# vghuy17ck1/svt-av1-psyex

Hardware: AMD Instinct MI355X
Metric: ME+RD-cost Mpixels/s (2160p10 preset-6) (higher is better)
Workload: dtype u8 SAD / i32 transforms; 1 GPU; 3840x2160 10-bit synthetic pan sequence, preset 6 (M6) search controls at qp 35; step = 16 pictures (4 current pictures x ref distance 1,2,4,8; R=2): open-loop ME of all 2040 b64 + full-pel pred + RD chain (64x64,32x32,16x16 DCT_DCT, 10-bit, b quantizer; qcoeff + recon + scalars written); 3 picture sets alternate from step to step

## Files before the change

svt-av1-psyex_amd/csrc/me_kernel.hip:

```cpp
#include <hip/hip_runtime.h>
#include <stdint.h>
#include <string.h>
#include "me_kernel.h"
#include "wave_ops.h"
#include "lds_dma.h"

#ifdef SVT_HIP_ME_PROFILE
struct Prof { uint32_t *acc; unsigned long long last; int step; };
#define SVT_HIP_ME_PROFILE_LDS (48 * 4)
#define PROF_DECL Prof prof_; prof_.acc = reinterpret_cast<uint32_t *>(g_lds + lay.total); if (threadIdx.x < 48) prof_.acc[threadIdx.x] = 0; prof_.last = __builtin_readcyclecounter(); prof_.step = 0; Prof *prof = &prof_
#define PROF_STEP(s) (prof->step = (s))
#define PROFS(i) PROF((i) + prof->step)
#define PROF(i) do { const unsigned long long t_ = __builtin_readcyclecounter(); if (threadIdx.x == 0) atomicAdd(&prof->acc[i], (uint32_t)(t_ - prof->last)); prof->last = t_; } while (0)
#define PROF_FLUSH(ptr) do { __builtin_amdgcn_fence(__ATOMIC_RELEASE, "wavefront"); if (threadIdx.x < 48) atomicAdd((unsigned long long *)(ptr) + threadIdx.x, (unsigned long long)prof->acc[threadIdx.x]); } while (0)
#define PROF_PARAM , Prof *prof
#define PROF_ARG , prof
#else
#define PROF_DECL do { } while (0)
#define PROF(i) do { } while (0)
#define PROFS(i) do { } while (0)
#define PROF_STEP(s) do { } while (0)
#define PROF_FLUSH(ptr) do { } while (0)
#define SVT_HIP_ME_PROFILE_LDS 0
#define PROF_PARAM
// ... 506 lines not shown
    constexpr int kArenaVec = kWinBytes / 16;
    int nt = 1;
    if (n1 <= kSmallVec && n0 + n1 <= kArenaVec) {
        nt = 2;
        if (n2 <= kSmallVec && n0 + n1 + n2 <= kArenaVec) {
            nt = 3;
            if (n3 <= kSmallVec && n0 + n1 + n2 + n3 <= kArenaVec) nt = 4;
        }
    }
    tile_load<0, 2>(read_tile(st, i), v);
    if (nt > 1) tile_load<2, 2>(read_tile(st, i + 1), v);
    if (nt > 2) tile_load<4, 2>(read_tile(st, i + 2), v);
    if (nt > 3) tile_load<6, 2>(read_tile(st, i + 3), v);
    return nt;
}
static_assert(kVecPerLane >= 8, "four small tiles of two slots each");

__device__ __forceinline__ void run_searches(Shared &sh PROF_PARAM) {
    St        &st   = sh.st;
    const int  nreq = (int)uni((uint32_t)st.nreq);
    V4         v[kVecPerLane];
    u64        key = (0xffffffull << 32) | 0xffffffffull;
    for (int t0 = 0;; t0 += kMaxTiles) {
        const int total = plan_tiles(st, nreq, t0), n = imin(total - t0, kMaxTiles);
        wave_sync();
        int nv[4] = {0, 0, 0, 0}, nvn[4] = {0, 0, 0, 0};
        int i = 0, nt = load_round(st, 0, n, v, nv);
        PROFS(24);
        while (nt) {
            {
                if (nv[0] > kSmallVec) tile_store<0, kVecPerLane>(sh, nv[0], 0, v);
                else {
                    tile_store<0, 2>(sh, nv[0], 0, v);
                    if (nt > 1) tile_store<2, 2>(sh, nv[1], nv[0], v);
                    if (nt > 2) tile_store<4, 2>(sh, nv[2], nv[0] + nv[1], v);
                    if (nt > 3) tile_store<6, 2>(sh, nv[3], nv[0] + nv[1] + nv[2], v);
                }
            }
            wave_sync();
            PROFS(32);
            const int nn = load_round(st, i + nt, n, v, nvn);
            PROF(22);
            int lds_vec = 0;
            for (int j = 0; j < nt; j++) {
                const TileGeo t = read_tile(st, i + j);
                const u64 k = tile_eval(sh, t, lds_vec * 16 PROF_ARG);
                key = k < key ? k : key;
                lds_vec += t.nvec;
                if (t.last) {
                    if (threadIdx.x == 0) st.req_key[t.req] = key;
                    key = (0xffffffull << 32) | 0xffffffffull;
                }
            }
            wave_sync();
            PROFS(40);
            i += nt;
            nt = nn;
#pragma unroll
            for (int j = 0; j < 4; j++) nv[j] = nvn[j];
        }
        if (t0 + kMaxTiles >= total) break;
        wave_sync();
    }
}

template <int NDW, int DEPTH>
__device__ __forceinline__ void direct_rows(uint8_t *arena, const uint8_t *src, int sp, int srs, const uint8_t *wp, long long wstep, int e0, int rows, int rows_max, uint32_t out[8]) {
    constexpr int NV = (NDW + 2 + 3) / 4, kRowsPerFlush = 64 / NDW;
    static_assert(NV & 1, "owners read their pieces back without bank conflicts");
    static_assert(DEPTH >= 1 && DEPTH <= 3, "steps in flight");
    const int lane = threadIdx.x;
    const uint8_t *pp[NV];
    int            pn[NV];
#pragma unroll
    for (int k = 0; k < NV; k++) {
        const int n = lane + 64 * k, owner = n / NV, part = n - owner * NV;
        const u64 base = ((u64)(uint32_t)__shfl((int)(uint32_t)((uintptr_t)wp >> 32), owner, 64) << 32) | (uint32_t)__shfl((int)(uint32_t)(uintptr_t)wp, owner, 64);
        pp[k] = reinterpret_cast<const uint8_t *>((uintptr_t)base) + 16 * part;
        pn[k] = __shfl(rows, owner, 64);
    }
    uint32_t a[8] = {0, 0, 0, 0, 0, 0, 0, 0};
    V4U v[DEPTH][NV];
    auto request = [&](V4U (&r)[NV], int step) {
#pragma unroll
        for (int k = 0; k < NV; k++) {
            if (step < pn[k]) r[k] = *reinterpret_cast<GV4U *>(reinterpret_cast<uintptr_t>(pp[k]));
            pp[k] += wstep;
        }
    };
#pragma unroll
    for (int dpt = 0; dpt < DEPTH; dpt++) {
#pragma unroll
        for (int k = 0; k < NV; k++) v[dpt][k] = V4U{0, 0, 0, 0};
        request(v[dpt], dpt);
    }
    u64 acc0 = 0, acc1 = 0;
    auto step = [&](V4U (&r)[NV], int t) {
#pragma unroll
        for (int k = 0; k < NV; k++) *reinterpret_cast<V4U *>(arena + 16 * (lane + 64 * k)) = r[k];
        wave_sync();
        request(r, t + DEPTH);
        if (t < rows) {
            const uint32_t *s = reinterpret_cast<const uint32_t *>(src + (e0 + t) * srs * sp);
            uint32_t sv[NDW], wv[4 * NV];
#pragma unroll
            for (int j = 0; j < NDW; j += 4) {
                const uint4 q = *reinterpret_cast<const uint4 *>(s + j);
                sv[j] = q.x; sv[j + 1] = q.y; sv[j + 2] = q.z; sv[j + 3] = q.w;
            }
#pragma unroll
            for (int k = 0; k < NV; k++) {
                const uint4 q = *reinterpret_cast<const uint4 *>(arena + 16 * (lane * NV + k));
                wv[4 * k] = q.x; wv[4 * k + 1] = q.y; wv[4 * k + 2] = q.z; wv[4 * k + 3] = q.w;
            }
#pragma unroll
            for (int j = 0; j < NDW; j++) {
                acc0 = __builtin_amdgcn_qsad_pk_u16_u8(((u64)wv[j + 1] << 32) | wv[j], sv[j], acc0);
                acc1 = __builtin_amdgcn_qsad_pk_u16_u8(((u64)wv[j + 2] << 32) | wv[j + 1], sv[j], acc1);
            }
        }
        if ((t + 1) % kRowsPerFlush == 0 || t + 1 == rows_max) {
#pragma unroll
            for (int i = 0; i < 4; i++) { a[i] += (uint32_t)((acc0 >> (16 * i)) & 0xFFFF); a[4 + i] += (uint32_t)((acc1 >> (16 * i)) & 0xFFFF); }
            acc0 = acc1 = 0;
        }
        wave_sync();
    };
    for (int t = 0; t < rows_max; t += DEPTH) {
        step(v[0], t);
        if (DEPTH >= 2 && t + 1 < rows_max) step(v[DEPTH >= 2 ? 1 : 0], t + 1);
        if (DEPTH >= 3 && t + 2 < rows_max) step(v[DEPTH >= 3 ? 2 : 0], t + 2);
    }
#pragma unroll
    for (int i = 0; i < 8; i++) out[i] = a[i];
}

__device__ __forceinline__ bool small_direct_ok(const St &st, int *q_total = nullptr) {
    const int lane = threadIdx.x, nreq = (int)uni((uint32_t)st.nreq);
    const Req &r0 = st.req[0];
    const int  bw = (int)uni(r0.bw), bh = (int)uni(r0.bh), rs = (int)uni(r0.rs), level = (int)uni(r0.level), stride = (int)uni((uint32_t)r0.stride);
    bool ok = true;
    int  per = 0;
    if (lane < nreq) {
        const Req &r = st.req[lane];
        const int  w = r.sa_w, h = r.sa_h;
        ok  = w > 0 && h > 0 && w * h <= kNarrowMaxPos && r.bw == bw && r.bh == bh && r.rs == rs && r.level == level && (int)r.stride == stride && !r.skip_even && !r.done;
        per = ((w + 7) >> 3) * h;
    }
    if (!__all(ok) || (bw != 32 && bw != 64) || nreq > kMaxReq || nreq <= 0) return false;
    const int q = (int)wave_sum_dpp((uint32_t)per);
    if (q_total) *q_total = q;
    return q <= kThreads;
}
template <int DEPTH = 1> __device__ __forceinline__ bool run_small_searches_direct(Shared &sh PROF_PARAM) {
    St       &st   = sh.st;
    const int lane = threadIdx.x, nreq = (int)uni((uint32_t)st.nreq);
    int Q = 0;
    if (!small_direct_ok(st, &Q)) return false;
    Q = (int)uni((uint32_t)Q);
    const Req &r0 = st.req[0];
    const int  bw = (int)uni(r0.bw), bh = (int)uni(r0.bh), rs = (int)uni(r0.rs), level = (int)uni(r0.level);
    {
        int per = 0;
        if (lane < nreq) per = ((st.req[lane].sa_w + 7) >> 3) * st.req[lane].sa_h;
        int incl = per;
#pragma unroll
        for (int o = 1; o < 32; o <<= 1) { const int t = __shfl_up(incl, o, 64); if ((lane & 31) >= o) incl += t; }
        if (lane < nreq) st.req_key[lane] = (u64)(uint32_t)(incl - per);
    }
    wave_sync();
    int       S        = imin(bh, (int)uni(div_by_rcp((uint32_t)kThreads, rcp_of((uint32_t)Q))));
    const int rows_per = (int)uni(div_by_rcp((uint32_t)(bh + S - 1), rcp_of((uint32_t)S)));
    S                  = (int)uni(div_by_rcp((uint32_t)(bh + rows_per - 1), rcp_of((uint32_t)rows_per)));
    uint32_t *sad = reinterpret_cast<uint32_t *>(LDS(sh.win));
    const uint8_t *src = src_view(sh, level);
    const int      sp  = (level == 2) ? kSrc64Pitch : (level == 1 ? kSrc32Pitch : kSrc16Pitch), srs = rs >> sh.cshift;
    const long long wstep = (long long)rs * (long long)(int)uni((uint32_t)r0.stride);
    const bool mine = lane < Q * S;
    int req = 0, y = 0, g = 0, e0 = 0, rows = 0, w = 1;
    const uint8_t *wp = nullptr;
    if (mine) {
        const int slice = (int)div_by_rcp((uint32_t)lane, rcp_of((uint32_t)Q)), q = lane - slice * Q;
        for (int r = 1; r < nreq; r++) req += q >= (int)(uint32_t)st.req_key[r] ? 1 : 0;
        const Req &r = st.req[req];
        w = r.sa_w;
        const int ng = (w + 7) >> 3, ql = q - (int)(uint32_t)st.req_key[req];
        y = (int)div_by_rcp((uint32_t)ql, rcp_of((uint32_t)ng)); g = ql - y * ng;
        e0   = slice * rows_per;
        rows = imin(e0 + rows_per, bh) - e0;
        wp   = r.win + (long long)y * r.stride + (long long)e0 * wstep + 8 * g;
    }
    uint32_t s8[8];
    PROF(26);
    if (bw == 64) direct_rows<16, DEPTH>(LDS(sh.win), src, sp, srs, wp, wstep, e0, rows, rows_per, s8);
    else direct_rows<8, DEPTH>(LDS(sh.win), src, sp, srs, wp, wstep, e0, rows, rows_per, s8);
    PROF(27);
    for (int p = lane; p < nreq * kNarrowMaxPos; p += kThreads) sad[p] = 0;
    wave_sync();
    if (mine) {
#pragma unroll
        for (int i = 0; i < 8; i++)
            if (8 * g + i < w) atomicAdd(&sad[req * kNarrowMaxPos + y * w + 8 * g + i], s8[i]);
    }
    wave_sync();
    PROF(23);
    for (int rq = 0; rq < nreq; rq++) {
        const int      wr = (int16_t)uni((uint32_t)st.req[rq].sa_w), hr = (int16_t)uni((uint32_t)st.req[rq].sa_h);
        const uint32_t k32 = wave_min_dpp(lane < wr * hr ? (sad[rq * kNarrowMaxPos + lane] << 6) | (uint32_t)lane : 0xFFFFFFFFu);
        const int      wl = (int)(k32 & 63u), wy = (int)uni(div_by_rcp((uint32_t)wl, rcp_of((uint32_t)wr))), wx = wl - wy * wr;
        if (lane == 0) st.req_key[rq] = ((u64)(k32 >> 6) << 32) | ((uint32_t)wy << 16) | (uint32_t)wx;
    }
    wave_sync();
    return true;
}

constexpr int kDenseKinds = SVT_HIP_ME_DENSE_KINDS;
__device__ __forceinline__ uint32_t dense_pack(int a, int b) { return (uint32_t)(uint16_t)a | ((uint32_t)(uint16_t)b << 16); }
__device__ __forceinline__ void dense_take(St &st, const MeDenseSlot *dl, int idx, int req, const SearchGeo &g, uint32_t &n_hit, uint32_t &n_miss) {
    if (!dl) return;
    const MeDenseSlot s = dl[idx];
    if (s.org == dense_pack(g.ox, g.oy) && s.size == dense_pack(g.sa_w, g.sa_h)) {
        st.req[req].done = 1;
        st.req_key[req]  = s.key == ~0ull ? ((0xffffffull << 32) | 0xffffffffull) : s.key;
        n_hit++;
    } else
        n_miss++;
}

__device__ __forceinline__ void push_req(St &st, const uint8_t *win, uint32_t stride, int sa_w, int sa_h, int bw, int bh, int rs,
                                         int level, int skip, int slot = -1) {
    Req &r      = st.req[slot >= 0 ? slot : st.nreq++];
    r.win       = win;
    r.stride    = stride;
    r.sa_w      = (int16_t)sa_w;
    r.sa_h      = (int16_t)sa_h;
    r.bw        = (uint8_t)bw;
    r.bh        = (uint8_t)bh;
    r.rs        = (uint8_t)rs;
    r.level     = (uint8_t)level;
    r.skip_even = (uint8_t)(skip && bw == 16 && bh <= 16);
    r.done      = 0;
}

__device__ __forceinline__ void push_hme_req(St &st, CParams &p, int level, CPlane &rp, int org_x, int org_y,
                                             int bw, int bh, int ox, int oy, int sa_w, int sa_h, int skip, int slot = -1) {
    const int full = (p.cfg.hme_search_method == 1);
    push_req(st, plane_at(rp, org_x + ox, org_y + oy), rp.stride, sa_w, sa_h, bw, full ? bh : (bh >> 1), full ? 1 : 2, level, skip, slot);
}


__device__ __forceinline__ void upd(u64 &best, uint32_t sad, uint32_t ord) {
    const u64 k = ((u64)sad << 32) | ord;
    best        = k < best ? k : best;
}

__device__ __attribute__((noinline)) void stage_clamped(uint8_t *win, const uint8_t *pix0, uint32_t stride, int min_x, int max_x, int min_y, int max_y, int wx0, int wy0,
                                                        int pitch, int rows) {
    for (int i = threadIdx.x; i < pitch * rows; i += kThreads) {
        const int row = i / pitch, cb = i - row * pitch;
        const int x = imin(imax(wx0 + cb, min_x), max_x), y = imin(imax(wy0 + row, min_y), max_y);
        win[row * pitch + cb] = pix0[x + (long long)y * stride];
    }
}

constexpr int kMeOrdBits = 12;
__device__ __forceinline__ void run_me_searches(Shared &sh, CParams &p, const MeReq *list, int count, uint32_t *bsad, uint32_t *bmv, int r0n PROF_PARAM) {
    const int lane = threadIdx.x;
    const int sub  = (p.cfg.me_search_method == 0);
    const int nrow = sub ? 4 : 8, rstep = sub ? 2 : 1;
    const int g = lane >> 4, pu = lane & 15;
    const int bx = (pu & 1) | ((pu >> 1) & 2), by = ((pu >> 1) & 1) | ((pu >> 2) & 2);
    const uint8_t *srow = &LDS(sh.src64)[bx * 16];
    for (int mi = 0; mi < count; mi++) {
        MeReq m;
        {
            const MeReq &mm = list[mi];
            m.pix0 = uni_ptr(mm.pix0); m.stride = uni(mm.stride);
            m.ox = (int16_t)uni((uint32_t)mm.ox); m.oy = (int16_t)uni((uint32_t)mm.oy); m.sa_w = (int16_t)uni((uint32_t)mm.sa_w); m.sa_h = (int16_t)uni((uint32_t)mm.sa_h);
            m.li = (uint8_t)uni(mm.li); m.ri = (uint8_t)uni(mm.ri); m.probe = 0; m.pad = 0;
            m.min_x = (int16_t)uni((uint32_t)mm.min_x); m.max_x = (int16_t)uni((uint32_t)mm.max_x); m.min_y = (int16_t)uni((uint32_t)mm.min_y); m.max_y = (int16_t)uni((uint32_t)mm.max_y);
        }
        u64 b8[4] = {~0ull, ~0ull, ~0ull, ~0ull}, b16 = ~0ull, b32 = ~0ull, b64 = ~0ull;
        const int W = m.sa_w, H = m.sa_h;
        int       tw = W, th = H;
        auto me_pitch = [](int shift, int ww) { return ((shift + ww - 1 + 64 + 15) & ~15) + 16; };
        auto wbytes = [&](int ww, int hh) { return (uint32_t)me_pitch(0, ww) * (uint32_t)(hh - 1 + 64); };
        while (th > 1 && (wbytes(tw, th) > (uint32_t)kWinBytes || tw * th > (1 << kMeOrdBits))) th = (th + 1) >> 1;
        while (tw > 8 && (wbytes(tw, th) > (uint32_t)kWinBytes || tw * th > (1 << kMeOrdBits))) tw = ((tw >> 1) + 7) & ~7;
        for (int y0 = 0; y0 < H; y0 += th)
            for (int x0 = 0; x0 < W; x0 += tw) {
                const int w = imin(tw, W - x0), h = imin(th, H - y0);
                const uint8_t *gwin  = m.pix0 + (m.ox + x0) + (long long)(m.oy + y0) * m.stride;
                const int pitch = me_pitch(0, w);
                const int rows        = h - 1 + 64;
                const int vec_per_row = pitch >> 4;
                lds_dma_after_stores();
                const int wx0 = m.ox + x0, wy0 = m.oy + y0;
                if (m.ox + x0 >= m.min_x && m.ox + x0 + w - 1 + 63 <= m.max_x && wy0 >= m.min_y && wy0 + rows - 1 <= m.max_y) {
                    lds_dma_window(gwin, m.stride, vec_per_row, rows, g_lds, sh.win);
                    lds_dma_wait();
                } else {
                    stage_clamped(LDS(sh.win), m.pix0, m.stride, m.min_x, m.max_x, m.min_y, m.max_y, wx0, wy0, pitch, rows);
                }
                wave_sync();
                PROF(46);
                const int ng = (w + 3) >> 2;
                uint32_t k8[4] = {~0u, ~0u, ~0u, ~0u}, k16 = ~0u, k32 = ~0u, k64 = ~0u;
                const int kshift = kMeOrdBits + sub;
                for (int y = 0; y < h; y += 4) {
                    const bool live = y + g < h;
                    const int  yy   = live ? y + g : h - 1;
                    const uint8_t *wrow = &LDS(sh.win)[(yy + by * 16) * pitch + bx * 16];
                    const uint32_t ord0 = (uint32_t)(yy * w);
                    for (int gq = 0; gq < ng; gq++) {
                        const uint8_t *wp = wrow + 4 * gq;
                        u64 acc[4] = {0, 0, 0, 0};
#pragma unroll
// ... 275 lines not shown
    else { y = (int)((key >> 16) & 0xFFFF); x = (int)(key & 0xFFFF); }
    if (!full) sad *= 2;
}

__device__ __forceinline__ void push_zz_req(St &st, CPlane &rp, int dx, int dy, int slot = -1) {
    push_req(st, plane_at(rp, (int)st.org_x + dx, (int)st.org_y + dy), rp.stride, 1, 1, (int)st.b64_w, (int)st.b64_h >> 1, 2, 2, 0, slot);
}

}


#ifndef SVT_ME_CTRL_PRIO
#define SVT_ME_CTRL_PRIO 2
#endif
#define CTRL_PRIO(x) __builtin_amdgcn_s_setprio(x)

constexpr size_t kPersistBytes = (offsetof(St, req) + 15) & ~(size_t)15;
template <int MODE>
__device__ __forceinline__ void me_b64_body(const MeBatchHeader *__restrict__ ghdr, const MeKernelParams *__restrict__ gparams, const uint32_t launch_flags) {
    St     &st = *reinterpret_cast<St *>(g_lds);
    constexpr bool kImports = MODE == kMeMid2 || MODE == kMeTail;
    typedef const SVT_CONST_AS MeBatchHeader CHeader;
    CHeader  &hdr = *(CHeader *)ghdr;
    const int tid = threadIdx.x;
    const int       cshift = (int)hdr.cshift;
    const bool      has_dense = hdr.dense != nullptr;
    const LdsLayout lay    = lds_layout((int)hdr.n_slot, cshift, has_dense ? 1 : 0, MODE);
    uint32_t *const bsad = reinterpret_cast<uint32_t *>(g_lds + lay.bsad);
    uint32_t *const bmv  = reinterpret_cast<uint32_t *>(g_lds + lay.bmv);
    const MeDenseSlot *const dense_lds = has_dense ? reinterpret_cast<const MeDenseSlot *>(g_lds + lay.dense) : nullptr;
    uint32_t n_hit = 0, n_miss = 0;
    Shared sh = {st, lay.src64, lay.src32, lay.src16, lay.win, cshift};

    uint32_t xcc = 0;
    asm volatile("s_getreg_b32 %0, hwreg(HW_REG_XCC_ID)" : "=s"(xcc));
    xcc &= 7;
    int queue_probe = 0;
    constexpr int kList = 0;
    const bool list_mode = (launch_flags & 1u) != 0;
    const uint32_t n_total = hdr.job_base[hdr.n_pictures];
    uint32_t share_next = 0, share_end = 0, share_step = 1;
    if (MODE != kMeFull && !list_mode) {
        if (gridDim.x >= SVT_HIP_ME_QUEUES) {
            const uint32_t q = blockIdx.x % SVT_HIP_ME_QUEUES;
            share_step = (gridDim.x - q + SVT_HIP_ME_QUEUES - 1) / SVT_HIP_ME_QUEUES;
            share_next = hdr.queue_begin[q] + blockIdx.x / SVT_HIP_ME_QUEUES;
            share_end  = hdr.queue_begin[q + 1];
        } else {
            share_step = gridDim.x; share_next = blockIdx.x; share_end = n_total;
        }
    }
    auto fetch_job = [&]() {
        int job = -1;
        if (list_mode) {
            const uint32_t n = __hip_atomic_load(&hdr.queue_head[SVT_HIP_ME_LIST_COUNT(kList)], __ATOMIC_RELAXED, __HIP_MEMORY_SCOPE_AGENT);
            if (__hip_atomic_load(&hdr.queue_head[SVT_HIP_ME_LIST_CURSOR(kList)], __ATOMIC_RELAXED, __HIP_MEMORY_SCOPE_AGENT) >= n) return job;
            const uint32_t k = atomicAdd(&hdr.queue_head[SVT_HIP_ME_LIST_CURSOR(kList)], 1u);
            if (k < n) job = (int)hdr.lists[kList][k];
            return job;
        }
        if (MODE != kMeFull) {
            if (share_next < share_end) { job = (int)share_next; share_next += share_step; }
            return job;
        }
        while (queue_probe < SVT_HIP_ME_QUEUES) {
            const int      q  = (int)((xcc + queue_probe) & 7);
            const uint32_t lo = hdr.queue_begin[q], hi = hdr.queue_begin[q + 1];
            if (lo < hi) {
                const uint32_t k = atomicAdd(&hdr.queue_head[q], 1u);
                if (lo + k < hi) { job = (int)(lo + k); break; }
            }
            queue_probe++;
        }
        return job;
    };
    auto stage_base = [&](int gjob) { return hdr.stage + (size_t)gjob * SVT_HIP_ME_STAGE_BYTES; };
    auto export_state = [&](int gjob) {
        uint4 *dst = reinterpret_cast<uint4 *>(stage_base(gjob));
        const uint4 *src = reinterpret_cast<const uint4 *>(g_lds);
        for (int i = tid; i < (int)(kPersistBytes / 16); i += kThreads) dst[i] = src[i];
    };
    static_assert(kPersistBytes + kMaxReq * (sizeof(Req) + sizeof(u64)) <= SVT_HIP_ME_STAGE_BYTES, "a block's record holds its state, its requests and their results");
    auto export_reqs = [&](int gjob) {
        uint4 *dst = reinterpret_cast<uint4 *>(stage_base(gjob) + kPersistBytes);
        const uint4 *src = reinterpret_cast<const uint4 *>(st.req);
        static_assert(sizeof(Req) == 24 && (kMaxReq * sizeof(Req)) % 16 == 0, "requests are copied as 16-byte words");
        for (int i = tid; i < (int)(kMaxReq * sizeof(Req) / 16); i += kThreads) dst[i] = src[i];
    };
    auto keys_of = [&](int gjob) { return reinterpret_cast<u64 *>(stage_base(gjob) + kPersistBytes + kMaxReq * sizeof(Req)); };
    PROF_DECL;

    for (;;) {
        int gjob = 0;
        if (tid == 0) gjob = fetch_job();
        gjob = __builtin_amdgcn_readfirstlane(gjob);
        if (gjob < 0) break;
        PROF(0);
        int pic = 0;
        while (pic + 1 < (int)hdr.n_pictures && (uint32_t)gjob >= hdr.job_base[pic + 1]) pic++;
        pic = __builtin_amdgcn_readfirstlane(pic);
        CParams &p = ((CParams *)gparams)[pic];
        auto &c = p.cfg;
        auto &d = p.desc;
        const int full_hme = (c.hme_search_method == 1);
        const int nl       = d.num_of_list_to_search;
        const bool mctf    = c.me_type == 1;
        const int job      = gjob - (int)hdr.job_base[pic];
        const uint32_t bxi = (uint32_t)job % p.w64, byi = p.row0 + (uint32_t)job / p.w64;
        const uint32_t b   = bxi + byi * p.w64;
        const int r0n      = d.num_of_ref_pic_to_search[0];
#define BEST_SAD(li, ri) (bsad + (((li) ? r0n : 0) + (ri)) * 85)
#define BEST_MV(li, ri) (bmv + (((li) ? r0n : 0) + (ri)) * 85)
        const int n_rows   = r0n + (nl > 1 ? d.num_of_ref_pic_to_search[1] : 0);
        uint32_t *const jflag = hdr.job_flags ? hdr.job_flags + gjob : nullptr;
        if constexpr (me_is_search(MODE)) {
            constexpr int lvl = MODE == kMeS1 ? 1 : 2, parts = lvl == 1 ? 3 : 5;
            static_assert(offsetof(St, req) == kPersistBytes && offsetof(St, nreq) >= kPersistBytes - 16, "nreq sits in the last 16-byte word of the record's head, the requests behind it");
            static_assert(kSrc32Pitch == 3 * 16 && kSrc64Pitch == 5 * 16, "a view row is its pieces and one piece of padding");
            lds_dma_after_stores();
            lds_dma_copy(stage_base(gjob) + kPersistBytes - 16, g_lds, (uint32_t)(kPersistBytes - 16), 1 + (int)(kMaxReq * sizeof(Req) / 16));
            const int ox = (int)(bxi * 64) >> (2 - lvl), oy = (int)(byi * 64) >> (2 - lvl), rstep = 1 << cshift, npiece = ((lvl == 1 ? 32 : 64) >> cshift) * parts;
            for (int b0 = 0; b0 < npiece; b0 += kThreads) {
                const int n = b0 + tid, row = n / parts, cc = n - row * parts;
                if (n < npiece && cc < parts - 1) lds_dma_load16(plane_at(p.cur.lvl[lvl], ox + cc * 16, oy + row * rstep), g_lds, (lvl == 1 ? lay.src32 : lay.src64) + (uint32_t)b0 * 16);
            }
            const uint32_t f = __hip_atomic_load(jflag, __ATOMIC_RELAXED, __HIP_MEMORY_SCOPE_AGENT);
            lds_dma_wait();
            if (f & SVT_HIP_ME_JOB_DEFERRED) continue;
        } else if constexpr (kImports) {
            static_assert(offsetof(St, req_key) % 16 == 0 && kPersistBytes <= offsetof(St, req) + 8 && offsetof(St, req) + 8 <= offsetof(St, req_key), "the record's parts land on 16-byte words of their own");
            static_assert(kSrc64Pitch == 5 * 16, "a view row is four pieces and one piece of padding");
            lds_dma_after_stores();
            lds_dma_copy(stage_base(gjob), g_lds, 0, (int)(kPersistBytes / 16));
            lds_dma_copy(reinterpret_cast<const uint8_t *>(keys_of(gjob)), g_lds, (uint32_t)offsetof(St, req_key), (int)(kMaxReq * sizeof(u64) / 16));
            if constexpr (MODE == kMeTail) {
                const int ox = (int)(bxi * 64), oy = (int)(byi * 64), rstep = 1 << cshift, npiece = (64 >> cshift) * 5;
                for (int b0 = 0; b0 < npiece; b0 += kThreads) {
                    const int n = b0 + tid, row = n / 5, cc = n - row * 5;
                    if (n < npiece && cc < 4) lds_dma_load16(plane_at(p.cur.lvl[2], ox + cc * 16, oy + row * rstep), g_lds, lay.src64 + (uint32_t)b0 * 16);
                }
            }
            const uint32_t f = __hip_atomic_load(jflag, __ATOMIC_RELAXED, __HIP_MEMORY_SCOPE_AGENT);
            if constexpr (MODE == kMeTail)
                for (int i = tid; i < n_rows * 85; i += kThreads) { bmv[i] = 0; bsad[i] = SVT_HIP_MAX_SAD_VALUE; }
            if (tid == 0) { st.nme = 0; st.nprobe = 0; }
            lds_dma_wait();
            if (f & SVT_HIP_ME_JOB_DEFERRED) continue;
        }
        if constexpr (me_is_search(MODE)) {
            PROF(24);
            wave_sync();
            PROF(25);
            if (st.nreq) {
                (void)run_small_searches_direct<SVT_HIP_ME_SEARCH_DEPTH>(sh PROF_ARG);
            }
            wave_sync();
            u64 *keys = keys_of(gjob);
            if (tid < kMaxReq) keys[tid] = st.req_key[tid];
            wave_sync();
            continue;
        }

        if constexpr (!kImports) {
        if (tid == 0) {
            st.b64_index = b;
            st.org_x = bxi * 64; st.org_y = byi * 64;
            st.b64_w = (uint32_t)(d.aligned_width - st.org_x) < 64 ? d.aligned_width - st.org_x : 64;
            st.b64_h = (uint32_t)(d.aligned_height - st.org_y) < 64 ? d.aligned_height - st.org_y : 64;
            st.hme_l0_sa.sa_min.width = (uint16_t)c.hme_l0_sa.sa_min.width; st.hme_l0_sa.sa_min.height = (uint16_t)c.hme_l0_sa.sa_min.height;
            st.hme_l0_sa.sa_max.width = (uint16_t)c.hme_l0_sa.sa_max.width; st.hme_l0_sa.sa_max.height = (uint16_t)c.hme_l0_sa.sa_max.height;
            st.nreq = 0; st.nme = 0; st.nprobe = 0;
        }
        for (int i = tid; i < 3 * 2 * 4 * 2 * 2; i += kThreads) { (&st.hx[0][0][0][0][0])[i] = 0; (&st.hy[0][0][0][0][0])[i] = 0; (&st.hs[0][0][0][0][0])[i] = 0; }
        if constexpr (MODE == kMeFull)
            for (int i = tid; i < n_rows * 85; i += kThreads) { bmv[i] = 0; bsad[i] = SVT_HIP_MAX_SAD_VALUE; }
        if (tid < 8) {
            const int li = tid >> 2, ri = tid & 3;
            st.do_ref[li][ri] = 1; st.hme_sad64[li][ri] = 0xFFFFFFFFull; st.sr_divisor[li][ri] = 1; st.zz_sad[li][ri] = ~0u;
            st.hme_sc_x[li][ri] = st.hme_sc_y[li][ri] = 0;
            for (int sri = 0; sri < 2; sri++) {
                PreHme &ph = st.prehme[li][ri][sri];
                ph.valid = 0; ph.col = ph.row = 0; ph.sad = 0; ph.sa_w = ph.sa_h = 0;
                st.performed_phme[li][ri][sri] = 0;
            }
        }
        }
        if ((MODE == kMeFull || MODE == kMeMid1) && has_dense && tid < n_rows * kDenseKinds)
            reinterpret_cast<uint4 *>(g_lds + lay.dense)[tid] = reinterpret_cast<const uint4 *>(hdr.dense)[((size_t)gjob * hdr.n_slot) * kDenseKinds + tid];
        const bool zz_on = (MODE == kMeFull || MODE == kMeMid1) && (c.me_early_exit_th || c.me_safe_limit_zz_th);
        const int  nzz   = zz_on ? r0n + ((nl > 1 && d.temporal_layer_index > 0) ? d.num_of_ref_pic_to_search[1] : 0) : 0;
        uint32_t   zz_sum[8] = {0, 0, 0, 0, 0, 0, 0, 0};
        {
            const int ox = (int)(bxi * 64), oy = (int)(byi * 64), rstep = 1 << cshift;
            const int bw64 = imin(64, (int)d.aligned_width - ox), bh64 = imin(64, (int)d.aligned_height - oy);
            if constexpr (!kImports)
            for (int i = tid; i < (64 >> cshift) * 4; i += kThreads) {
                const int row = i >> 2, cc = i & 3;
                uint4 v; memcpy(&v, plane_at(p.cur.lvl[2], ox + cc * 16, oy + row * rstep), 16);
                if constexpr (MODE != kMeMid1) *reinterpret_cast<uint4 *>(&LDS(sh.src64)[row * kSrc64Pitch + cc * 16]) = v;
                const int y = row * rstep, x = cc * 16;
                if (nzz && !(y & 1) && y < bh64 && x < bw64) {
                    const bool whole = x + 8 < bw64;
#pragma unroll
                    for (int k = 0; k < 8; k++)
                        if (k < nzz) {
                            const int li = k < r0n ? 0 : 1, ri = k < r0n ? k : k - r0n;
                            uint4 w; memcpy(&w, plane_at(p.ref[li][ri].lvl[2], ox + x, oy + y), 16);
                            uint32_t a = __builtin_amdgcn_sad_u8(v.x, w.x, zz_sum[k]);
                            a = __builtin_amdgcn_sad_u8(v.y, w.y, a);
                            if (whole) { a = __builtin_amdgcn_sad_u8(v.z, w.z, a); a = __builtin_amdgcn_sad_u8(v.w, w.w, a); }
                            zz_sum[k] = a;
                        }
                }
            }
            if constexpr (MODE == kMeFull) {
                for (int i = tid; i < (32 >> cshift) * 2; i += kThreads) {
                    const int row = i >> 1, cc = i & 1;
                    uint4 v; memcpy(&v, plane_at(p.cur.lvl[1], (ox >> 1) + cc * 16, (oy >> 1) + row * rstep), 16);
                    *reinterpret_cast<uint4 *>(&LDS(sh.src32)[row * kSrc32Pitch + cc * 16]) = v;
                }
                for (int i = tid; i < (16 >> cshift); i += kThreads) {
                    uint4 v; memcpy(&v, plane_at(p.cur.lvl[0], ox >> 2, (oy >> 2) + i * rstep), 16);
                    *reinterpret_cast<uint4 *>(&LDS(sh.src16)[i * kSrc16Pitch]) = v;
                }
            }
        }
#pragma unroll
        for (int k = 0; k < 8; k++)
            if (k < nzz) {
                const uint32_t t = wave_sum_dpp(zz_sum[k]);
                if (tid == 0) st.req_key[k] = (u64)t << 32;
            }
        wave_sync();

        PROF(1);
        auto zz_pre = [&]() {
            if (tid == 0) st.nreq = 0;
        };
        auto zz_post = [&]() {
            const int  li = (tid >> 2) & 1, ri = tid & 3;
            const bool valid = tid < 8 && li < nl && ri < d.num_of_ref_pic_to_search[li];
            const bool srch  = valid && searched(p, li);
            const u64  smask = __ballot(srch);
            uint32_t   z = 0xFFFFFFFFu;
            if (srch) {
                const int k = __popcll(smask & ((1ull << tid) - 1ull));
                z = (uint32_t)(st.req_key[k] >> 32) << 1;
                z = (z * 64 * 64) / (st.b64_w * st.b64_h);
                st.zz_sad[li][ri] = z;
            }
            const uint32_t best = wave_min_dpp(z);
            if (d.temporal_layer_index > 0 && best < c.zz_sad_th && valid && ri >= 1)
                if ((uint32_t)((z - best) * 100) > (uint32_t)(c.zz_sad_pct * best)) st.do_ref[li][ri] = 0;
            if (c.me_safe_limit_zz_th) {
                wave_sync();
                const bool limit = d.hierarchical_levels > 0 && nl == 2 && d.temporal_layer_index >= d.hierarchical_levels &&
                    d.similar_brightness_refs && st.zz_sad[0][0] < c.me_safe_limit_zz_th && st.zz_sad[1][0] < c.me_safe_limit_zz_th;
                if (limit && valid && ri >= 1) st.do_ref[li][ri] = 0;
            }
        };
        auto prehme_pre = [&](int bi) {
            const int  l_lo = c.prehme_l1_early_exit ? bi : 0, l_hi = c.prehme_l1_early_exit ? bi + 1 : nl;
            const int  li = (tid >> 3) & 1, ri = (tid >> 1) & 3, sri = tid & 1;
            const bool mine = tid < 16 && li >= l_lo && li < l_hi && ri < d.num_of_ref_pic_to_search[li];
            bool       push = false;
            if (mine) {
                st.ph_req[li][ri][sri] = 0;
                if (searched(p, li)) {
                    PreHme &ph = st.prehme[li][ri][sri];
                    bool    handled = false;
                    if (c.me_early_exit_th && st.zz_sad[li][ri] < c.me_early_exit_th) { ph.col = ph.row = 0; ph.sad = 0; ph.valid = 1; handled = true; }
                    if (!handled && c.prehme_l1_early_exit) {
                        const PreHme &q = st.prehme[0][ri][sri];
                        if (li == 1 && q.valid && (q.sad < 32 * 32 || (iabs(q.col) < 16 && iabs(q.row) < 16))) {
                            ph.col = (int16_t)-q.col; ph.row = (int16_t)-q.row; ph.sad = q.sad; ph.valid = 1; handled = true;
                        }
                    }
                    if (!handled && !st.do_ref[li][ri]) { ph.col = ph.row = 0; ph.sad = 0xFFFFFFFFu; handled = true; }
                    push = !handled;
                }
            }
            const u64 mask = __ballot(push);
            const int slot = __popcll(mask & ((1ull << tid) - 1ull));
            if (push) {
                PreHme &ph = st.prehme[li][ri][sri];
                CPlane &rp = p.ref[li][ri].lvl[0];
                const int ox16 = (int16_t)st.org_x >> 2, oy16 = (int16_t)st.org_y >> 2;
                const SearchGeo sg = prehme_geometry(p, li, ri, sri, st.org_x, st.org_y);
                push_hme_req(st, p, 0, rp, ox16, oy16, (int)st.b64_w >> 2, (int)st.b64_h >> 2, sg.ox, sg.oy, sg.sa_w, sg.sa_h, c.prehme_skip_search_line, slot);
                st.ph_req[li][ri][sri] = (uint8_t)(slot + 1);
                dense_take(st, dense_lds, (((li ? r0n : 0) + ri) * kDenseKinds + sri), slot, sg, n_hit, n_miss);
                ph.col = (int16_t)sg.ox; ph.row = (int16_t)sg.oy;
                st.performed_phme[li][ri][sri] = 1;
            }
            if (tid == 0) st.nreq = __popcll(mask);
        };
        auto prehme_post = [&](int bi) {
            const int  l_lo = c.prehme_l1_early_exit ? bi : 0, l_hi = c.prehme_l1_early_exit ? bi + 1 : nl;
            const int  li = (tid >> 3) & 1, ri = (tid >> 1) & 3, sri = tid & 1;
            const bool mine = tid < 16 && li >= l_lo && li < l_hi && ri < d.num_of_ref_pic_to_search[li];
            const int  k = mine ? st.ph_req[li][ri][sri] : 0;
            if (k) {
                PreHme &ph = st.prehme[li][ri][sri];
                uint32_t sad; int x, y;
                key_to_result(st.req_key[k - 1], full_hme, sad, x, y);
                ph.sad = sad;
                ph.col = (int16_t)((int16_t)(x + ph.col) * 4);
// ... 245 lines not shown
                { const uint32_t q = (uint32_t)(int)sa_w / st.sr_divisor[li][ri]; sa_w = (int16_t)(((q > 1u ? q : 1u) + 7) & ~7u); }
                { const uint32_t q = (uint32_t)(int)sa_h / st.sr_divisor[li][ri]; sa_h = (int16_t)(q > 3u ? q : 3u); }
                const int16_t h0 = sa_h, w0 = sa_w;
                u64 best_hme_sad = ~0ull;
                if (c.me_early_exit_th) {
                    if (st.zz_sad[li][ri] < c.me_early_exit_th / 6) sa_w = sa_h = 1;
                } else {
                    int accurate = 1;
                    const int k2 = st.c00_req[li][ri];
                    if (k2) {
                        const uint32_t zero = (uint32_t)(st.req_key[k2 - 2] >> 32) << 1;
                        const uint32_t hme  = (uint32_t)(st.req_key[k2 - 1] >> 32) << 1;
                        if (zero <= hme) cx = cy = 0;
                        best_hme_sad = hme;
                        if (cx == 0 && cy == 0) accurate = 0;
                    }
                    if (c.enable_me_sr_adjustment == 2) {
                        if ((accurate && best_hme_sad < 24 * 24) || (d.is_ref && st.hme_sad64[li][ri] < 24 * 24)) sa_h = (int16_t)(sa_h / 2);
                        if ((li || ri) && BEST_SAD(0, 0)[0] < 5000 && sa_h == h0 && sa_w == w0) { sa_h = (int16_t)(sa_h >> 1); sa_w = (int16_t)(sa_w >> 1); }
                    }
                }
                m.pix0 = plane_at(rp, (int)st.org_x, (int)st.org_y); m.stride = rp.stride;
                m.min_x = (int16_t)(-rp.org_x - (int)st.org_x); m.max_x = (int16_t)(rp.width + rp.org_x - 1 - (int)st.org_x);
                m.min_y = (int16_t)(-rp.org_y - (int)st.org_y); m.max_y = (int16_t)(rp.height + rp.org_y - 1 - (int)st.org_y);
                m.li = (uint8_t)li; m.ri = (uint8_t)ri; m.pad = 0;
                m.sa_w = sa_w; m.sa_h = sa_h;
                m.ox = cx; m.oy = cy;
                m.probe = (c.me_8x8_var_enabled && sa_w * sa_h > 24) ? 1 : 0;
            }
            const bool probe = mine && m.probe;
            const u64  mask = __ballot(mine), pmask = __ballot(probe), below = (1ull << tid) - 1ull;
            if (mine) st.me[__popcll(mask & below)] = m;
            if (probe) { MeReq pr = m; pr.sa_w = pr.sa_h = 1; st.me_probe[__popcll(pmask & below)] = pr; }
            if (tid == 0) { st.nme = __popcll(mask); st.nprobe = __popcll(pmask); }
        };
        auto main_pre = [&]() {
            if (tid < 64) {
                const int pic_w = (int16_t)d.aligned_width, pic_h = (int16_t)d.aligned_height;
                for (int i = 0; i < st.nme; i++) {
                    const MeReq m = st.me[i];
                    int16_t sa_w = m.sa_w, sa_h = m.sa_h;
                    const int cx = m.ox, cy = m.oy;
                    if (m.probe) {
                        const uint32_t mean = BEST_SAD(m.li, m.ri)[0] / 64;
                        const int32_t  dd   = (int32_t)BEST_SAD(m.li, m.ri)[21 + tid] - (int32_t)mean;
                        const uint32_t var  = wave_sum((uint32_t)(dd * dd)) / 64;
                        if (var > c.me_sr_mult2_th) { sa_w = (int16_t)((imax(1, sa_w * 3 / 2) + 7) & ~7); sa_h = (int16_t)imax(1, sa_h * 3 / 2); }
                        if (var < c.me_sr_div4_th) { sa_w = (int16_t)((imax(1, sa_w >> 2) + 7) & ~7); sa_h = (int16_t)imax(3, imax(1, sa_h >> 2)); }
                        else if (var < c.me_sr_div2_th) { sa_w = (int16_t)((imin(sa_w, sa_w >> 1) + 7) & ~7); sa_h = (int16_t)imax(3, imin(sa_h, sa_h >> 1)); }
                    }
                    int ox = (int16_t)(cx - (sa_w >> 1)), oy = (int16_t)(cy - (sa_h >> 1)), w = sa_w, h = sa_h;
                    clip_axis((int16_t)st.org_x, ox, w, 63, pic_w);
                    w = (w < 8) ? w : (w & ~7);
                    clip_axis((int16_t)st.org_y, oy, h, 63, pic_h);
                    if (tid == 0) { MeReq &o = st.me[i]; o.ox = (int16_t)ox; o.oy = (int16_t)oy; o.sa_w = (int16_t)w; o.sa_h = (int16_t)h; }
                }
            }
        };

        enum { kZz, kPrehme, kL0, kL1, kL2, kC00, kProbe, kMain, kEnd };
#ifdef SVT_ME_ABLATE
        if (SVT_ME_ABLATE == 1) continue;
#endif
        const int n_prehme = c.prehme_l1_early_exit ? nl : 1, n_l0 = l0_dep ? 2 : 1, n_group = me_dep ? 2 : 1;
        if constexpr (MODE == kMeMid1 || MODE == kMeMid2) {
            const bool hme_on = c.enable_hme_flag;
            bool defer = false;
            uint32_t flags = 0;
            if constexpr (MODE == kMeMid1) {
                auto pending = [&]() { return __any(tid < st.nreq && !st.req[tid].done); };
                if (c.me_early_exit_th || c.me_safe_limit_zz_th) { zz_pre(); wave_sync(); zz_post(); wave_sync(); }
                if (c.prehme_enable) {
                    for (int b2 = 0; b2 < n_prehme; b2++) {
                        prehme_pre(b2); wave_sync();
                        if (pending()) { defer = true; break; }
                        prehme_post(b2);
                        if (b2 + 1 < n_prehme) wave_sync();
                    }
                    if (!defer) { prehme_final(); wave_sync(); }
                }
                if (!defer && hme_on && c.enable_hme_level0_flag)
                    for (int b2 = 0; b2 < n_l0; b2++) {
                        l0_pre(b2); wave_sync();
                        if (pending()) { defer = true; break; }
                        l0_post(b2); wave_sync();
                    }
                if (!defer) {
                    if (hme_on && c.enable_hme_level1_flag) lvl_pre(1);
                    else if (tid == 0) st.nreq = 0;
                    wave_sync();
                }
            } else {
                flags = __hip_atomic_load(jflag, __ATOMIC_RELAXED, __HIP_MEMORY_SCOPE_AGENT);
                if (hme_on && c.enable_hme_level1_flag) { lvl_post(1); wave_sync(); }
                if (hme_on && c.enable_hme_level2_flag) lvl_pre(2);
                else if (tid == 0) st.nreq = 0;
                wave_sync();
            }
            if (!defer && st.nreq && !small_direct_ok(st)) defer = true;
            if (defer) {
                if (tid == 0) {
                    *jflag = SVT_HIP_ME_JOB_DEFERRED;
                    hdr.lists[0][atomicAdd(&hdr.queue_head[SVT_HIP_ME_LIST_COUNT(0)], 1u)] = (uint32_t)gjob;
                }
            } else {
                export_state(gjob);
                export_reqs(gjob);
                if (tid == 0) *jflag = flags;
            }
            wave_sync();
            continue;
        }
        if constexpr (MODE == kMeTail) {
            if (c.enable_hme_flag && c.enable_hme_level2_flag) { lvl_post(2); wave_sync(); }
        }
        int step = MODE == kMeTail ? kC00 : kZz, bi = 0;
        PROF(2);
        while (step != kEnd) {
            bool run = true;
            CTRL_PRIO(SVT_ME_CTRL_PRIO);
            switch (step) {
            case kZz: run = c.me_early_exit_th || c.me_safe_limit_zz_th; if (run) zz_pre(); break;
            case kPrehme: run = c.prehme_enable; if (run) prehme_pre(bi); break;
            case kL0: run = c.enable_hme_flag && c.enable_hme_level0_flag; if (run) l0_pre(bi); break;
            case kL1: run = c.enable_hme_flag && c.enable_hme_level1_flag; if (run) lvl_pre(1); break;
            case kL2: run = c.enable_hme_flag && c.enable_hme_level2_flag; if (run) lvl_pre(2); break;
            case kC00: if (bi == 0) centre(); c00_pre(bi); break;
            case kProbe: probe_pre(bi); break;
            default: main_pre(); break;
            }
#ifdef SVT_ME_ABLATE
            if (SVT_ME_ABLATE == 2 && step == kC00) break;
            if (SVT_ME_ABLATE >= 10 && step == SVT_ME_ABLATE - 10) break;
            if (SVT_ME_ABLATE == 4 && run && step < kProbe) { step = step == kPrehme ? kL0 : step + 1; bi = 0; continue; }
            if (SVT_ME_ABLATE == 5 && run && step < kProbe) st.nreq = 0;
#endif
            if (run) {
                CTRL_PRIO(0);
                wave_sync();
                PROF(step == kMain ? 20 : 6 + step);
                if (step == kC00 && bi == 0 && st.tf_exit) { step = kEnd; continue; }
                if constexpr (MODE == kMeTail) {
                    if (step == kC00) {
                        c00_sads(sh);
                        PROF(18);
                    } else if (step == kProbe) {
                        probe_sads(sh, p, bsad, bmv, r0n PROF_ARG);
                    } else {
                        run_me_searches(sh, p, st.me, st.nme, bsad, bmv, r0n PROF_ARG);
                    }
                } else if (step < kProbe) {
                    PROF_STEP(step);
                    if (st.nreq) {
                        if (!run_small_searches_direct(sh PROF_ARG)) run_searches(sh PROF_ARG);
                    }
                } else {
                    const bool   probe = step == kProbe;
                    const MeReq *list  = probe ? st.me_probe : st.me;
                    const int    count = probe ? st.nprobe : st.nme;
                    run_me_searches(sh, p, list, count, bsad, bmv, r0n PROF_ARG);
                }
                PROF(step == kProbe ? 3 : step == kMain ? 4 : 19);
            }
            CTRL_PRIO(SVT_ME_CTRL_PRIO);
            switch (step) {
            case kZz: if (run) zz_post(); step = kPrehme; break;
            case kPrehme:
                if (run) prehme_post(bi);
                if (run && bi + 1 < n_prehme) { bi++; break; }
                if (run) prehme_final();
                step = kL0; bi = 0;
                break;
            case kL0:
                if (run) l0_post(bi);
                if (run && bi + 1 < n_l0) { bi++; break; }
                step = kL1; bi = 0;
                break;
            case kL1: if (run) lvl_post(1); step = kL2; break;
            case kL2: if (run) lvl_post(2); step = kC00; break;
            case kC00: step = kProbe; break;
            case kProbe: step = kMain; break;
            default:
                if (bi + 1 < n_group) { bi++; step = kC00; } else step = kEnd;
                break;
            }
            CTRL_PRIO(0);
            wave_sync();
            PROF(5);
        }


#ifdef SVT_ME_ABLATE
        if (SVT_ME_ABLATE == 2 || SVT_ME_ABLATE == 3 || SVT_ME_ABLATE >= 10) continue;
#endif
        if (c.enable_hme_flag && c.enable_me_hme_ref_pruning && !mctf) {
            for (int r = 0; r < 8; r++) {
                const int li = r >> 2, ri = r & 3;
                if (li >= nl || ri >= d.num_of_ref_pic_to_search[li]) continue;
                const u64 t = st.do_ref[li][ri] ? (u64)wave_sum(BEST_SAD(li, ri)[21 + (tid & 63)]) : (u64)SVT_HIP_MAX_SAD_VALUE * 64;
                if ((tid & 63) == 0) st.hme_sad64[li][ri] = t;
            }
            wave_sync();
            {
                const uint16_t th = c.prune_ref_if_me_sad_dev_bigger_than_th;
                if (th != 0xFFFF) {
                    const int  li = (tid >> 2) & 1, ri = tid & 3;
                    const bool slot = tid < 8;
                    const u64  hs = slot ? st.hme_sad64[li][ri] : ~0ull;
                    const u64  best = (u64)wave_min_dpp((uint32_t)(hs < 0xFFFFFFFFull ? hs : 0xFFFFFFFFull));
                    if (slot && ri >= 1 && (hs - best) * 100 > (u64)th * best) st.do_ref[li][ri] = 0;
                }
            }
            wave_sync();
        }

        PROF(13);
        {
          if (!mctf) {
            const uint32_t n_pu = p.n_pu;
            uint8_t  *o_total = p.res.total_me_candidate_index + (size_t)b * n_pu;
            uint32_t *o_mv    = p.res.me_mv_array + (size_t)b * n_pu * d.max_refs;
            uint8_t  *o_cand  = p.res.me_candidate_array + (size_t)b * n_pu * d.max_cand;
            const int r0 = d.num_of_ref_pic_to_search[0], r1 = d.num_of_ref_pic_to_search[1];
            auto use_pu = [&](int nn) { return d.enable_me_16x16 ? (d.enable_me_8x8 || nn < 21) : nn < 5; };
            auto pack   = [](unsigned dir, unsigned i0, unsigned i1, unsigned l0, unsigned l1) {
                return (uint8_t)((dir & 3) | ((i0 & 3) << 2) | ((i1 & 3) << 4) | ((l0 & 1) << 6) | ((l1 & 1) << 7));
            };
            uint32_t *l_mv    = reinterpret_cast<uint32_t *>(LDS(sh.win));
            uint8_t  *l_cand  = LDS(sh.win) + 4 * n_pu * d.max_refs;
            uint8_t  *l_total = l_cand + n_pu * d.max_cand;
            const int stage_dwords = (int)(4 * n_pu * d.max_refs + n_pu * d.max_cand + n_pu + 3) >> 2;
            static_assert(kWinBytes >= 85 * (4 * SVT_HIP_MAX_LISTS * SVT_HIP_MAX_REFS + 32 + 1), "the result rows of one block fit the arena");
            for (int i = tid; i < stage_dwords; i += kThreads) reinterpret_cast<uint32_t *>(LDS(sh.win))[i] = 0;
            wave_sync();
            for (int n = tid; n < d.max_number_of_pus_per_sb; n += kThreads) {
                const int use = use_pu(n);
                const int row = (n > 4) ? c_z_to_raster[n] : n;
                uint8_t first = 0;
                auto put_cand = [&](int idx, uint8_t v) { l_cand[row * d.max_cand + idx] = v; if (idx == 0) first = v; };
                uint32_t  nls = nl;
                if (r0 == 1 && r1 == 0) {
                    const int pu   = c_z_to_raster[n];
                    st.me_dist[pu] = BEST_SAD(0, 0)[n];
                    if (use) l_total[pu] = 1;
                    if (st.do_ref[0][0] && use) { put_cand(0, pack(0, 0, 0, 0, 0)); l_mv[pu * d.max_refs] = BEST_MV(0, 0)[n]; }
                } else if (r0 == 1 && r1 == 1) {
                    const int     pu = c_z_to_raster[n];
                    const uint8_t d0 = st.do_ref[0][0], d1 = (nls == 1) ? 0 : st.do_ref[1][0];
                    if (nls < 2 || !st.do_ref[1][0]) nls = 1;
                    const uint32_t prune_th = (d0 && d1) ? (uint32_t)c.prune_me_candidates_th : 0;
                    uint8_t  blk[2] = {d0, d1};
                    uint8_t  off = 0;
                    const uint32_t s0 = BEST_SAD(0, 0)[n], s1 = BEST_SAD(1, 0)[n];
                    const uint32_t best = (d0 && d1) ? (s0 < s1 ? s0 : s1) : (d0 ? s0 : s1);
                    st.me_dist[pu] = best;
                    if (use) l_total[pu] = 1;
                    int min_list = -1;
                    if (c.use_best_unipred_cand_only && blk[0] && blk[1]) min_list = s0 < s1 ? 0 : 1;
                    for (uint32_t li = 0; li < nls && (use || off == 0); li++) {
                        if (!blk[li]) continue;
                        if (prune_th > 0) {
                            const uint32_t dev = (BEST_SAD(li, 0)[n] - best) * 100;
                            if (dev > best * prune_th) { blk[li] = 0; continue; }
                        }
                        if (min_list != -1 && min_list != (int)li) {
                            if (use) l_mv[pu * d.max_refs + (li ? d.max_l0 : 0)] = BEST_MV(li, 0)[n];
                            continue;
                        }
                        if (use) {
                            put_cand(off, pack(li, 0, 0, li == 0 ? li : 24, li == 1 ? li : 24));
                            l_mv[pu * d.max_refs + (li ? d.max_l0 : 0)] = BEST_MV(li, 0)[n];
                        }
                        off++;
                    }
                    if (blk[0] && blk[1] && use) { put_cand(off, pack(2, 0, 0, 0, 1)); l_total[pu] = (uint8_t)(off + 1); }
                } else {
                    const int pu = (n > 4) ? c_z_to_raster[n] : n;
                    uint8_t   off = 0;
                    uint8_t   blk[2][4] = {{0, 0, 0, 0}, {0, 0, 0, 0}};
                    const uint32_t prune_th = (uint32_t)c.prune_me_candidates_th;
                    uint32_t       best     = ~0u;
                    for (uint32_t li = 0; li < nls; li++)
                        for (int ri = 0; ri < d.num_of_ref_pic_to_search[li]; ri++) {
                            blk[li][ri] = st.do_ref[li][ri];
                            if (blk[li][ri]) best = BEST_SAD(li, ri)[n] < best ? BEST_SAD(li, ri)[n] : best;
                        }
                    st.me_dist[pu] = best;
                    for (uint32_t li = 0; li < nls && (use || off == 0); li++)
                        for (int ri = 0; ri < d.num_of_ref_pic_to_search[li] && (use || off == 0); ri++) {
                            if (!blk[li][ri]) continue;
                            if (prune_th > 0) {
                                const uint32_t dev = (BEST_SAD(li, ri)[n] - best) * 100;
                                if (dev > best * prune_th) { blk[li][ri] = 0; continue; }
                            }
                            if (use) {
                                put_cand(off, pack(li, ri, ri, li == 0 ? li : 24, li == 1 ? li : 24));
                                l_mv[pu * d.max_refs + (li ? d.max_l0 : 0) + ri] = BEST_MV(li, ri)[n];
                            }
                            off++;
                        }
                    if (nls == 2 && use) {
                        for (int a = 0; a < r0; a++)
                            for (int bb = 0; bb < r1; bb++) {
                                if (d.only_l_bwd && (a > 0 || bb > 0)) continue;
                                if (blk[0][a] && blk[1][bb]) put_cand(off++, pack(2, a, bb, 0, 1));
                            }
                        if (!d.only_l_bwd) {
// ... 311 lines not shown
```

Measured before the change: 43690 Mpixels/s.

## Add ring-buffered row-streaming SAD path for small narrow ME searches

Adds a ring-based direct search path for small search areas (width ≤8, height ≤3, row step ≤2). Each lane owns a request/row-slice, streams reference rows through LDS with loads kept in flight, and accumulates SADs with qsad_pk across the three vertical offsets. Partial sums are combined across slices with DPP reductions. The search-only mode can also skip the small_direct_ok qualification check when its requests are trusted, while the full-pipeline caller keeps the old path by default. This aims to cut redundant reference loads and LDS traffic, at the cost of more register pressure and a reliance on requests actually meeting the assumed constraints.

```diff
diff --git a/svt-av1-psyex_amd/csrc/me_kernel.hip b/svt-av1-psyex_amd/csrc/me_kernel.hip
--- a/svt-av1-psyex_amd/csrc/me_kernel.hip
+++ b/svt-av1-psyex_amd/csrc/me_kernel.hip
@@ -682,17 +682,167 @@
     if (q_total) *q_total = q;
     return q <= kThreads;
 }
-template <int DEPTH = 1> __device__ __forceinline__ bool run_small_searches_direct(Shared &sh PROF_PARAM) {
+template <int NDW, int DEPTH>
+__device__ __forceinline__ void ring_rows(uint8_t *arena, const uint8_t *src, int sp, int srs, const St &st, int nreq, int lg, int S, int rows_per, int bh, int rs, int sa_h,
+                                          long long stride, uint32_t (&a)[3][8]) {
+    constexpr int NV = (NDW + 2 + 3) / 4, kRowsPerFlush = 64 / NDW;
+    static_assert(NV & 1, "owners read their pieces back without bank conflicts");
+    static_assert(DEPTH >= 1 && DEPTH <= 3, "steps in flight");
+    const int lane = threadIdx.x, gmask = (1 << lg) - 1;
+    const int steps_max = rs * (rows_per - 1) + sa_h;
+    const uint8_t *pp[NV];
+    int            pn[NV];
+#pragma unroll
+    for (int k = 0; k < NV; k++) {
+        const int  n = lane + 64 * k, owner = n / NV, part = n - owner * NV, orq = owner >> lg, osl = owner & gmask;
+        const bool act = orq < nreq && osl < S;
+        const int  oe0 = osl * rows_per, orows = imin(oe0 + rows_per, bh) - oe0;
+        pn[k] = act ? rs * (orows - 1) + sa_h : 0;
+        pp[k] = st.req[act ? orq : 0].win + (long long)(oe0 * rs) * stride + 16 * part;
+    }
+    const int  req = lane >> lg, slice = lane & gmask, e0 = slice * rows_per;
+    const int  rows = (req < nreq && slice < S) ? imin(e0 + rows_per, bh) - e0 : 0;
+    V4U v[DEPTH][NV];
+    auto request = [&](V4U (&r)[NV], int step) {
+#pragma unroll
+        for (int k = 0; k < NV; k++) {
+            if (step < pn[k]) r[k] = *reinterpret_cast<GV4U *>(reinterpret_cast<uintptr_t>(pp[k]));
+            pp[k] += stride;
+        }
+    };
+#pragma unroll
+    for (int dpt = 0; dpt < DEPTH; dpt++) {
+#pragma unroll
+        for (int k = 0; k < NV; k++) v[dpt][k] = V4U{0, 0, 0, 0};
+        request(v[dpt], dpt);
+    }
+#pragma unroll
+    for (int y = 0; y < 3; y++)
+#pragma unroll
+        for (int i = 0; i < 8; i++) a[y][i] = 0;
+    u64 acc[3][2] = {{0, 0}, {0, 0}, {0, 0}};
+    auto step = [&](V4U (&r)[NV], int j) {
+#pragma unroll
+        for (int k = 0; k < NV; k++) *reinterpret_cast<V4U *>(arena + 16 * (lane + 64 * k)) = r[k];
+        wave_sync();
+        request(r, j + DEPTH);
+        uint32_t wv[4 * NV];
+#pragma unroll
+        for (int k = 0; k < NV; k++) {
+            const uint4 q = *reinterpret_cast<const uint4 *>(arena + 16 * (lane * NV + k));
+            wv[4 * k] = q.x; wv[4 * k + 1] = q.y; wv[4 * k + 2] = q.z; wv[4 * k + 3] = q.w;
+        }
+#pragma unroll
+        for (int y = 0; y < 3; y++) {
+            const int dd = j - y, t = rs == 2 ? dd >> 1 : dd;
+            if (y < sa_h && dd >= 0 && (rs == 1 || !(dd & 1)) && t < rows_per) {
+                if (t < rows) {
+                    const uint32_t *s = reinterpret_cast<const uint32_t *>(src + (e0 + t) * srs * sp);
+                    uint32_t sv[NDW];
+#pragma unroll
+                    for (int c = 0; c < NDW; c += 4) {
+                        const uint4 q = *reinterpret_cast<const uint4 *>(s + c);
+                        sv[c] = q.x; sv[c + 1] = q.y; sv[c + 2] = q.z; sv[c + 3] = q.w;
+                    }
+#pragma unroll
+                    for (int c = 0; c < NDW; c++) {
+                        acc[y][0] = __builtin_amdgcn_qsad_pk_u16_u8(((u64)wv[c + 1] << 32) | wv[c], sv[c], acc[y][0]);
+                        acc[y][1] = __builtin_amdgcn_qsad_pk_u16_u8(((u64)wv[c + 2] << 32) | wv[c + 1], sv[c], acc[y][1]);
+                    }
+                }
+                if ((t + 1) % kRowsPerFlush == 0 || t + 1 == rows_per) {
+#pragma unroll
+                    for (int i = 0; i < 4; i++) { a[y][i] += (uint32_t)((acc[y][0] >> (16 * i)) & 0xFFFF); a[y][4 + i] += (uint32_t)((acc[y][1] >> (16 * i)) & 0xFFFF); }
+                    acc[y][0] = acc[y][1] = 0;
+                }
+            }
+        }
+        wave_sync();
+    };
+    for (int j = 0; j < steps_max; j += DEPTH) {
+        step(v[0], j);
+        if (DEPTH >= 2 && j + 1 < steps_max) step(v[DEPTH >= 2 ? 1 : 0], j + 1);
+        if (DEPTH >= 3 && j + 2 < steps_max) step(v[DEPTH >= 3 ? 2 : 0], j + 2);
+    }
+}
+
+template <int DEPTH> __device__ __forceinline__ void run_ring_searches(Shared &sh, int nreq, int bw, int bh, int rs, int level, int sa_h PROF_PARAM) {
+    St       &st   = sh.st;
+    const int lane = threadIdx.x;
+    int lg = 0;
+    while ((2 << lg) * nreq <= kThreads) lg++;
+    const int S0 = imin(bh, 1 << lg), rows_per = (int)uni(div_by_rcp((uint32_t)(bh + S0 - 1), rcp_of((uint32_t)S0)));
+    const int S  = (int)uni(div_by_rcp((uint32_t)(bh + rows_per - 1), rcp_of((uint32_t)rows_per)));
+    const uint8_t *src = src_view(sh, level);
+    const int      sp  = (level == 2) ? kSrc64Pitch : (level == 1 ? kSrc32Pitch : kSrc16Pitch), srs = rs >> sh.cshift;
+    const long long stride = (long long)(int)uni((uint32_t)st.req[0].stride);
+    uint32_t a[3][8];
+    PROF(26);
+    if (bw == 64) ring_rows<16, DEPTH>(LDS(sh.win), src, sp, srs, st, nreq, lg, S, rows_per, bh, rs, sa_h, stride, a);
+    else ring_rows<8, DEPTH>(LDS(sh.win), src, sp, srs, st, nreq, lg, S, rows_per, bh, rs, sa_h, stride, a);
+    PROF(27);
+#define SVT_RING_SUM(cond, expr)                                                  \
+    if (cond) {                                                                   \
+        _Pragma("unroll") for (int y = 0; y < 3; y++)                             \
+            _Pragma("unroll") for (int i = 0; i < 8; i++) { const uint32_t v = a[y][i]; a[y][i] = v + (uint32_t)(expr); } \
+    }
+    SVT_RING_SUM(lg >= 1, __builtin_amdgcn_mov_dpp((int)v, 0xB1 , 0xF, 0xF, true))
+    SVT_RING_SUM(lg >= 2, __builtin_amdgcn_mov_dpp((int)v, 0x4E , 0xF, 0xF, true))
+    SVT_RING_SUM(lg >= 3, __builtin_amdgcn_mov_dpp((int)v, 0x141 , 0xF, 0xF, true))
+    SVT_RING_SUM(lg >= 4, __builtin_amdgcn_mov_dpp((int)v, 0x140 , 0xF, 0xF, true))
+    SVT_RING_SUM(lg >= 5, __shfl_xor((int)v, 16, 64))
+    SVT_RING_SUM(lg >= 6, __shfl_xor((int)v, 32, 64))
+#undef SVT_RING_SUM
+    PROF(23);
+    const int req = lane >> lg;
+    if (req < nreq && (lane & ((1 << lg) - 1)) == 0) {
+        const int w = st.req[req].sa_w;
+        uint32_t  best = 0xFFFFFFFFu;
+#pragma unroll
+        for (int y = 0; y < 3; y++)
+#pragma unroll
+            for (int i = 0; i < 8; i++)
+                if (y < sa_h && i < w) best = umin(best, (a[y][i] << 6) | (uint32_t)(y * w + i));
+        const int wl = (int)(best & 63u), wy = (int)div_by_rcp((uint32_t)wl, rcp_of((uint32_t)w)), wx = wl - wy * w;
+        st.req_key[req] = ((u64)(best >> 6) << 32) | ((uint32_t)wy << 16) | (uint32_t)wx;
+    }
+    wave_sync();
+}
+
+#ifndef SVT_HIP_ME_DIRECT_RING
+#define SVT_HIP_ME_DIRECT_RING 1
+#endif
+#ifndef SVT_HIP_ME_DIRECT_RING_FULL
+#define SVT_HIP_ME_DIRECT_RING_FULL 0
+#endif
+#ifndef SVT_HIP_ME_DIRECT_TRUST
+#define SVT_HIP_ME_DIRECT_TRUST 1
+#endif
+template <int DEPTH = 1, bool QUALIFIED = false, bool RING = true> __device__ __forceinline__ bool run_small_searches_direct(Shared &sh PROF_PARAM) {
     St       &st   = sh.st;
     const int lane = threadIdx.x, nreq = (int)uni((uint32_t)st.nreq);
-    int Q = 0;
-    if (!small_direct_ok(st, &Q)) return false;
-    Q = (int)uni((uint32_t)Q);
+    if constexpr (!(QUALIFIED && SVT_HIP_ME_DIRECT_TRUST)) {
+        if (!small_direct_ok(st)) return false;
+    }
     const Req &r0 = st.req[0];
     const int  bw = (int)uni(r0.bw), bh = (int)uni(r0.bh), rs = (int)uni(r0.rs), level = (int)uni(r0.level);
+    int per = 0;
+    if constexpr (RING && SVT_HIP_ME_DIRECT_RING) {
+        const int h0 = (int)uni((uint32_t)r0.sa_h);
+        bool alike = true;
+        if (lane < nreq) {
+            const int w = st.req[lane].sa_w, h = st.req[lane].sa_h;
+            alike = w <= 8 && h == h0;
+            per   = ((w + 7) >> 3) * h;
+        }
+        if (h0 <= 3 && rs <= 2 && __all(alike)) {
+            run_ring_searches<DEPTH>(sh, nreq, bw, bh, rs, level, h0 PROF_ARG);
+            return true;
+        }
+    } else if (lane < nreq)
+        per = ((st.req[lane].sa_w + 7) >> 3) * st.req[lane].sa_h;
+    const int Q = (int)wave_sum_dpp((uint32_t)per);
     {
-        int per = 0;
-        if (lane < nreq) per = ((st.req[lane].sa_w + 7) >> 3) * st.req[lane].sa_h;
         int incl = per;
 #pragma unroll
         for (int o = 1; o < 32; o <<= 1) { const int t = __shfl_up(incl, o, 64); if ((lane & 31) >= o) incl += t; }
@@ -1274,7 +1424,7 @@
             wave_sync();
             PROF(25);
             if (st.nreq) {
-                (void)run_small_searches_direct<SVT_HIP_ME_SEARCH_DEPTH>(sh PROF_ARG);
+                (void)run_small_searches_direct<SVT_HIP_ME_SEARCH_DEPTH, MODE == kMeS1>(sh PROF_ARG);
             }
             wave_sync();
             u64 *keys = keys_of(gjob);
@@ -1826,7 +1976,7 @@
                 } else if (step < kProbe) {
                     PROF_STEP(step);
                     if (st.nreq) {
-                        if (!run_small_searches_direct(sh PROF_ARG)) run_searches(sh PROF_ARG);
+                        if (!run_small_searches_direct<1, false, SVT_HIP_ME_DIRECT_RING_FULL != 0>(sh PROF_ARG)) run_searches(sh PROF_ARG);
                     }
                 } else {
                     const bool   probe = step == kProbe;
```

After: 45040 Mpixels/s (median of 6 runs). 1.03x the previous value.
